# hccho2/Tacotron-Wavenet-Vocoder-Korean

Hardware: AMD Instinct MI355X
Metric: WaveNet autoregressive audio samples/sec at 24 kHz, batch=8 (higher is better)
Workload: dtype f32

## Files before the change

### tacotron-wavenet-vocoder-korean_amd/csrc/twv_wavenet_xcd.hip

```cpp
#include <hip/hip_runtime.h>
#include <stdint.h>
#include <string>
#include <type_traits>
#include "../../include/twv_amd.h"
#include "twv_layout.hpp"
#include "twv_math.hpp"
#include "twv_dev.hpp"
#include "twv_dpp.hpp"
#include "twv_categorical.hpp"
#include "twv_xcd.hpp"

using namespace twv;

#ifndef TWV_CHAIN_PAD
#define TWV_CHAIN_PAD 0
#endif
#ifndef TWV_WATCHDOG_LOG2
#define TWV_WATCHDOG_LOG2 21
#endif
#define TWV_STR2(x) #x
#define TWV_STR(x) TWV_STR2(x)
namespace {

typedef __attribute__((address_space(1))) unsigned long long gu64;
#define LDSU64(i) (((__attribute__((address_space(3))) volatile unsigned long long*)lds)[(i)])

typedef unsigned u32x2v __attribute__((ext_vector_type(2)));
typedef unsigned u32x4s __attribute__((ext_vector_type(4)));
constexpr int kAuxLoad = (int)(16u | 0x80000000u), kAuxStore = 0;
#ifndef TWV_XCD_KF
#define TWV_XCD_KF 1
#endif

__device__ __forceinline__ unsigned long long xb_load(rsrc_t rs, int uword, int lword)
{
    asm volatile("" ::: "memory");
    const u32x2v v = __builtin_amdgcn_raw_buffer_load_b64(rs, lword * 8, uword * 8, kAuxLoad);
    return ((unsigned long long)v.y << 32) | (unsigned long long)v.x;
}
__device__ __forceinline__ u32x4s xb_load2(rsrc_t rs, int uword, int lpair)
{
    asm volatile("" ::: "memory");
    return __builtin_amdgcn_raw_buffer_load_b128(rs, lpair * 16, uword * 8, kAuxLoad);
}
template <bool BAR> __device__ __forceinline__ unsigned long long xb_load_t(rsrc_t rs, int uword, int lword)
{
    if (BAR) asm volatile("" ::: "memory");
    return xb_load(rs, uword, lword);
}
__device__ __forceinline__ unsigned long long xbm_load(rsrc_t rs, int uword, int lword) { return xb_load_t<true>(rs, uword, lword); }
__device__ __forceinline__ u32x4s xbm_load2(rsrc_t rs, int uword, int lpair)
{
    asm volatile("" ::: "memory");
    return xb_load2(rs, uword, lpair);
}
__device__ __forceinline__ void xb_store(rsrc_t rs, int uword, int lword, unsigned tag, float v)
{
    __builtin_amdgcn_raw_buffer_store_b64(u32x2v{__float_as_uint(v), tag}, rs, lword * 8, uword * 8, kAuxStore);
    asm volatile("" ::: "memory");
}
__device__ __forceinline__ void xb_store2(rsrc_t rs, int uword, int lane, unsigned tag, float va, float vb)
{
    const u32x4s d = {__float_as_uint(va), tag, __float_as_uint(vb), tag};
    __builtin_amdgcn_raw_buffer_store_b128(d, rs, lane * 16, uword * 8, kAuxStore);
    asm volatile("s_nop 1" ::"v"(d) : "memory");
}
__device__ __forceinline__ unsigned g_tag(unsigned long long q) { return (unsigned)(q >> 32); }
__device__ __forceinline__ float g_val(unsigned long long q) { return __uint_as_float((unsigned)q); }

struct Poll {
    rsrc_t rs;
    int* status;
    int it;
    bool dead;
};
template <bool BAR = false>
__device__ __forceinline__ bool poll_tick(Poll& p, int code)
{
    if (p.dead) return false;
    if (((++p.it) & 63) == 0) {
        if (xb_load_t<BAR>(p.rs, (int)XcdExch::CTRL + 1, 0) != 0ull) { p.dead = true; return false; }
        if (p.it > (1 << TWV_WATCHDOG_LOG2)) {
            atomicMax(p.status, code);
            xb_store(p.rs, (int)XcdExch::CTRL + 1, 0, 1u, 0.0f);
            p.dead = true;
            return false;
        }
    }
    return true;
}
__device__ __forceinline__ void nap_until(unsigned long long target)
{
#pragma nounroll
    for (int i = 0; i < 4096 && __builtin_amdgcn_s_memtime() < target; ++i) __builtin_amdgcn_s_sleep(8);
}

__device__ __forceinline__ int lane_of_z(int k) { return ((k & 2) ? 16 : 0) + 2 * (k >> 2) + (k & 1); }
__device__ __forceinline__ int lane_of_x(int j) { return j < 16 ? j : 16 + j; }

struct ChainRegs { float wc[32]; float bd; };
__device__ __forceinline__ void dot32_dpp_chain_lo(const float (&w)[16], float xa, float init, float (&c)[4])
{
    float c0 = init, c1, c2, c3;
    asm volatile(
        "s_nop 1\n" TWV_ALIGN8
        "v_fmac_f32_dpp %0, %4, %5 row_newbcast:0 row_mask:0xf bank_mask:0xf\n"
        "v_mul_f32_dpp %1, %4, %6 row_newbcast:1 row_mask:0xf bank_mask:0xf\n"
        "v_mul_f32_dpp %2, %4, %7 row_newbcast:2 row_mask:0xf bank_mask:0xf\n"
        "v_mul_f32_dpp %3, %4, %8 row_newbcast:3 row_mask:0xf bank_mask:0xf\n"
        "v_fmac_f32_dpp %0, %4, %9 row_newbcast:4 row_mask:0xf bank_mask:0xf\n"
        "v_fmac_f32_dpp %1, %4, %10 row_newbcast:5 row_mask:0xf bank_mask:0xf\n"
        "v_fmac_f32_dpp %2, %4, %11 row_newbcast:6 row_mask:0xf bank_mask:0xf\n"
        "v_fmac_f32_dpp %3, %4, %12 row_newbcast:7 row_mask:0xf bank_mask:0xf\n"
        "v_fmac_f32_dpp %0, %4, %13 row_newbcast:8 row_mask:0xf bank_mask:0xf\n"
        "v_fmac_f32_dpp %1, %4, %14 row_newbcast:9 row_mask:0xf bank_mask:0xf\n"
        "v_fmac_f32_dpp %2, %4, %15 row_newbcast:10 row_mask:0xf bank_mask:0xf\n"
        "v_fmac_f32_dpp %3, %4, %16 row_newbcast:11 row_mask:0xf bank_mask:0xf\n"
        "v_fmac_f32_dpp %0, %4, %17 row_newbcast:12 row_mask:0xf bank_mask:0xf\n"
        "v_fmac_f32_dpp %1, %4, %18 row_newbcast:13 row_mask:0xf bank_mask:0xf\n"
        "v_fmac_f32_dpp %2, %4, %19 row_newbcast:14 row_mask:0xf bank_mask:0xf\n"
        "v_fmac_f32_dpp %3, %4, %20 row_newbcast:15 row_mask:0xf bank_mask:0xf"
        : "+v"(c0), "=&v"(c1), "=&v"(c2), "=&v"(c3)
        : "v"(xa), "v"(w[0]), "v"(w[1]), "v"(w[2]), "v"(w[3]), "v"(w[4]), "v"(w[5]), "v"(w[6]), "v"(w[7]), "v"(w[8]), "v"(w[9]), "v"(w[10]), "v"(w[11]), "v"(w[12]), "v"(w[13]), "v"(w[14]), "v"(w[15]));
    c[0] = c0; c[1] = c1; c[2] = c2; c[3] = c3;
}
__device__ __forceinline__ float dot32_dpp_chain_hi(const float (&w)[16], float xb, const float (&c)[4])
{
    float c0 = c[0], c1 = c[1], c2 = c[2], c3 = c[3];
    asm volatile(
        TWV_ALIGN8
        "v_fmac_f32_dpp %0, %4, %5 row_newbcast:0 row_mask:0xf bank_mask:0xf\n"
        "v_fmac_f32_dpp %1, %4, %6 row_newbcast:1 row_mask:0xf bank_mask:0xf\n"
        "v_fmac_f32_dpp %2, %4, %7 row_newbcast:2 row_mask:0xf bank_mask:0xf\n"
        "v_fmac_f32_dpp %3, %4, %8 row_newbcast:3 row_mask:0xf bank_mask:0xf\n"
        "v_fmac_f32_dpp %0, %4, %9 row_newbcast:4 row_mask:0xf bank_mask:0xf\n"
        "v_fmac_f32_dpp %1, %4, %10 row_newbcast:5 row_mask:0xf bank_mask:0xf\n"
        "v_fmac_f32_dpp %2, %4, %11 row_newbcast:6 row_mask:0xf bank_mask:0xf\n"
        "v_fmac_f32_dpp %3, %4, %12 row_newbcast:7 row_mask:0xf bank_mask:0xf\n"
        "v_fmac_f32_dpp %0, %4, %13 row_newbcast:8 row_mask:0xf bank_mask:0xf\n"
        "v_fmac_f32_dpp %1, %4, %14 row_newbcast:9 row_mask:0xf bank_mask:0xf\n"
        "v_fmac_f32_dpp %2, %4, %15 row_newbcast:10 row_mask:0xf bank_mask:0xf\n"
        "v_fmac_f32_dpp %3, %4, %16 row_newbcast:11 row_mask:0xf bank_mask:0xf\n"
        "v_fmac_f32_dpp %0, %4, %17 row_newbcast:12 row_mask:0xf bank_mask:0xf\n"
        "v_fmac_f32_dpp %1, %4, %18 row_newbcast:13 row_mask:0xf bank_mask:0xf\n"
        "v_fmac_f32_dpp %2, %4, %19 row_newbcast:14 row_mask:0xf bank_mask:0xf\n"
        "v_fmac_f32_dpp %3, %4, %20 row_newbcast:15 row_mask:0xf bank_mask:0xf"
        : "+v"(c0), "+v"(c1), "+v"(c2), "+v"(c3)
        : "v"(xb), "v"(w[0]), "v"(w[1]), "v"(w[2]), "v"(w[3]), "v"(w[4]), "v"(w[5]), "v"(w[6]), "v"(w[7]), "v"(w[8]), "v"(w[9]), "v"(w[10]), "v"(w[11]), "v"(w[12]), "v"(w[13]), "v"(w[14]), "v"(w[15]));
    return (c0 + c1) + (c2 + c3);
}

#define XSTAMP(cond_, slot_) do { if ((INSTR & 1) && a.prof != nullptr && b == a.prof_stream && t < a.prof_steps && lane == 0 && (cond_)) a.prof[(long long)t * 64 + (slot_)] = wall_clock64(); } while (0)

#define WACC_DECL() unsigned long long wacc_[6] = {0, 0, 0, 0, 0, 0}, w0_ = 0, wt0_ = 0; if (INSTR & 4) wt0_ = __builtin_amdgcn_s_memtime()
#define WACC_T0() do { if (INSTR & 4) w0_ = __builtin_amdgcn_s_memtime(); } while (0)
#define WACC_T1(i_) do { if (INSTR & 4) wacc_[i_] += __builtin_amdgcn_s_memtime() - w0_; } while (0)
constexpr int kTraceStep = 2000;
#define WTRACE(cond_, slot_) do { if ((INSTR & 4) && a.prof != nullptr && t == kTraceStep && (cond_) && lane == 0) a.prof[2048 + (slot_)] = wall_clock64(); } while (0)
#define WACC_OUT(prof_, slot_, wave_) do { if ((INSTR & 4) && (prof_) != nullptr && (slot_) >= 0 && lane == 0) {                 \
        unsigned long long* o_ = (prof_) + (((slot_) * 8 + (wave_)) * 8);                                                        \
        o_[0] = __builtin_amdgcn_s_memtime() - wt0_;                                                                             \
        o_[1] = wacc_[0]; o_[2] = wacc_[1]; o_[3] = wacc_[2]; o_[4] = wacc_[3]; o_[5] = wacc_[4]; o_[6] = wacc_[5]; } } while (0)
#define XMARK(role_, stage_) do { if ((INSTR & 1) && lane == 0) xb_store(rs, (int)XcdExch::MARK + (role_) * 8 + (int)(threadIdx.x >> 6), 0, (unsigned)t + 1u, (float)(stage_)); } while (0)

enum { ROLE_CHAIN = 0, ROLE_SERVICE = 1, ROLE_SKIP0 = 2, ROLE_CONV0 = 10 };
constexpr int kXcdStreamsPerXcd = kXcdStreams / 8;

struct XArgs {
    XcdLaunch p;
    int n_lc_wg, lc_lpw;
    int n_conv1;
    int total_roles;
};

template <int NS> struct XStreams { rsrc_t rs[NS]; int b[NS]; };
__device__ __forceinline__ rsrc_t exch_rsrc(const XcdLaunch& a, int b)
{
    return __builtin_amdgcn_make_buffer_rsrc(a.exch + (long long)b * XcdExch::WORDS, 0, (int)(XcdExch::WORDS * 8), 0x00020000);
}
struct XLazyRs { const XcdLaunch* a; int xcc, ns; __device__ __forceinline__ rsrc_t operator[](int k) const { return exch_rsrc(*a, xcc + 8 * (k < ns ? k : 0)); } };
struct XLazyB { int xcc, ns; __device__ __forceinline__ int operator[](int k) const { return xcc + 8 * (k < ns ? k : 0); } };
template <int NS> struct XStreamsLazy { XLazyRs rs; XLazyB b; };
constexpr int kSkipLdsWords = 32 * 64;
constexpr int kConvLdsFloats = 16 * 64 + 64;

constexpr int kChainLpw = 5;
template <int INSTR, bool ALL, bool FORCED, bool SEG1, bool TWOSEG, int NC, bool ONEHOT = false, bool HEAD = false, bool CONT = false>
__device__ __forceinline__ void chain_role(const XArgs& xa, int b, rsrc_t rs)
{
    const XcdLaunch& a = xa.p;
    const Layout& L = a.lay;
    const int w = __builtin_amdgcn_readfirstlane(threadIdx.x >> 6), lane = threadIdx.x & 63;
    const int NL = L.NL, T = a.T;
    const bool use_bias = L.use_bias != 0, has_gc = L.G > 0, has_lc = L.L > 0;
    constexpr bool forced = FORCED;
    constexpr int kLayerWaves = kXcdSeg0Layers / kChainLpw;
    const int l0 = (SEG1 ? kXcdSeg0Layers : 0) + kChainLpw * w;
    const int lw0 = kChainLpw * w;
    const int cap = (HEAD || w >= kLayerWaves) ? 0 : kChainLpw;
    int nl = NL - l0;
    nl = nl < 0 ? 0 : (nl > cap ? cap : nl);
    const int nlc = NC >= 0 ? NC : nl;
    const bool next_has = (l0 + nl < NL);
    constexpr bool head = HEAD;
    const bool to_seg1 = TWOSEG && !SEG1 && w == kLayerWaves - 1 && next_has;
    constexpr bool two_seg = TWOSEG;
    if (nl == 0 && !head) return;
    const int oc = dpp_conv_out(lane), od = dpp_dense_out(lane);
    const ActCoef coef = act_coef(lane >= 32);
    float* stb = a.state + (long long)b * L.state_stride;
    Poll pl{rs, a.status, 0, false};
    constexpr int O_WD = 2048;
    constexpr int O_WH = kXcdChainHalfTiles;

    float wlo[kChainLpw - 1][16], whi[kChainLpw][16], bdi[kChainLpw];
#pragma unroll
    for (int i = 0; i < kChainLpw; ++i) {
        if (!HEAD && i < nl) {
            const f32x4* src = reinterpret_cast<const f32x4*>(a.P + L.off_xl + (long long)(l0 + i) * kXcdXlFloats) + lane;
#pragma unroll
            for (int q = 0; q < 4; ++q) {
                const f32x4 lo = src[q * 64], hi = src[(4 + q) * 64];
                if (i == 0) LDS4((O_WH >> 2) + (w * 4 + q) * 64 + lane) = lo;
                else { wlo[i > 0 ? i - 1 : 0][4 * q] = lo.x; wlo[i > 0 ? i - 1 : 0][4 * q + 1] = lo.y; wlo[i > 0 ? i - 1 : 0][4 * q + 2] = lo.z; wlo[i > 0 ? i - 1 : 0][4 * q + 3] = lo.w; }
                whi[i][4 * q] = hi.x; whi[i][4 * q + 1] = hi.y; whi[i][4 * q + 2] = hi.z; whi[i][4 * q + 3] = hi.w;
            }
#pragma unroll
            for (int q = 0; q < 4; ++q) LDS4((O_WD >> 2) + ((lw0 + i) * 4 + q) * 64 + lane) = src[(8 + q) * 64];
            const f32x4 v = src[12 * 64];
            bdi[i] = dense_bias_init(lane, use_bias ? v.y : 0.0f);
        }
    }
    float wcz[32];
    float ha = 0.0f, hb = 0.0f, first_in = 0.0f, b2v = 0.0f, s_lnl = 0.0f, s_tq = 0.0f, samp = 0.0f;
    float cp[4] = {0.0f, 0.0f, 0.0f, 0.0f};
    int q_prev = 0, q_valid = 0, samp_q = 0, first_q = 0;
    float w0row = 0.0f;
    double u_next = 0.0;
    const int chx = dpp_dense_out(lane);
    const bool sampler = head && !forced;
    const bool is15 = (lane & 15) == 15;
    auto causal_prepare = [&]() {
        const float t1 = __int_as_float(__builtin_amdgcn_update_dpp(0, __float_as_int(ha), 0x101, 0xf, 0xf, true));
        const float b0 = __int_as_float(__builtin_amdgcn_update_dpp(0, __float_as_int(hb), 0x150, 0xf, 0xf, true));
        ha = is15 ? b0 : t1;
        hb = __int_as_float(__builtin_amdgcn_update_dpp(0, __float_as_int(hb), 0x101, 0xf, 0xf, true));
        causal_partial_dpp(wcz, ha, hb, cp);
// ... 354 lines not shown
    Poll pl{rs, a.status, 0, false};
    constexpr int kReg = 4, kLds = BIG ? 3 : 0, kSlots = kReg + kLds;
    const int NLDS = BIG ? (NL > 8 * kReg ? NL - 8 * kReg : 0) : 0;
    int nown = 0, nlds = 0;
#pragma unroll
    for (int i = 0; i < kReg; ++i) if (NLDS + s + 8 * i < NL) nown = i + 1;
#pragma unroll
    for (int j = 0; j < kLds; ++j) if (s + 8 * j < NLDS) nlds = j + 1;
    if (nown == 0 && nlds == 0) return;
    Tile t0[kReg];
    unsigned dil[kSlots], roff[kSlots], pos0[kSlots];
    int lay_of[kSlots];
    float bfg[kSlots], gcv[kSlots];
#pragma unroll
    for (int i = 0; i < kSlots; ++i) {
        dil[i] = 1; roff[i] = 0; pos0[i] = 0; bfg[i] = 0.0f; gcv[i] = 0.0f;
        const bool is_lds = i < kLds;
        const int l = is_lds ? s + 8 * i : NLDS + s + 8 * (i - kLds);
        const bool have = is_lds ? i < nlds : (i - kLds) < nown;
        lay_of[i] = have ? l : -1;
        if (have) {
            const float* src = a.P + L.off_layer0 + (long long)l * L.layer_stride + LayerOff::T0;
            if (is_lds) copy_tile_to_lds(l * (kTile / 4), src, lane);
            else load_tile(t0[i - kLds < 0 ? 0 : i - kLds], src, lane);
            dil[i] = (unsigned)pmeta[l]; roff[i] = (unsigned)pmeta[64 + l]; pos0[i] = (unsigned)ringpos[l];
            if (use_bias) bfg[i] = a.P[L.off_layer0 + (long long)l * L.layer_stride + LayerOff::BFG + lane];
            if (has_gc) gcv[i] = a.cond[XH_WORDS + ((long long)b * NL + l) * 64 + lane];
        }
    }
    auto addend = [&](int i, float pre, float lcv) __attribute__((always_inline)) -> float {
        float v = pre;
        if (use_bias) v = v + bfg[i];
        if (has_gc) v = v + gcv[i];
        if (has_lc) v = v + lcv;
        return v;
    };
    const int n16 = lane & 15;
    auto tap0 = [&](int i, unsigned t, float& xa_, float& xb_) __attribute__((always_inline)) {
        const unsigned slot = ring_slot(pos0[i], t, dil[i]);
        const unsigned long long* p = reinterpret_cast<const unsigned long long*>(ring + roff[i] + slot * 32);
        const unsigned long long qa = __hip_atomic_load((gu64*)(p + (n16 >> 1)), __ATOMIC_RELAXED, __HIP_MEMORY_SCOPE_AGENT);
        const unsigned long long qb = __hip_atomic_load((gu64*)(p + 8 + (n16 >> 1)), __ATOMIC_RELAXED, __HIP_MEMORY_SCOPE_AGENT);
        xa_ = __uint_as_float((n16 & 1) ? (unsigned)(qa >> 32) : (unsigned)qa);
        xb_ = __uint_as_float((n16 & 1) ? (unsigned)(qb >> 32) : (unsigned)qb);
    };
    auto dot_slot = [&](int i, float oa, float ob) __attribute__((always_inline)) -> float {
        if (i < kLds) return dot32_dpp_lds(lay_of[i] * (kTile / 4), lane, oa, ob);
        return dot32_dpp(t0[i - kLds < 0 ? 0 : i - kLds].w, oa, ob);
    };
#pragma unroll
    for (int i = 0; i < kSlots; ++i) {
        if (lay_of[i] >= 0) {
            const int l = lay_of[i];
            float xa_, xb_;
            tap0(i, 0u, xa_, xb_);
            const float pre = dot_slot(i, xa_, xb_);
            const float lcv = has_lc ? stb[L.st_lcprev + l * 64 + lane] : 0.0f;
            xb_store(rs, (int)XcdExch::PG + l * 64, lane, 1u, addend(i, pre, lcv));
        }
    }
    for (int t = 0; t < T && !pl.dead; ++t) {
        asm volatile(".p2align 6");
        const unsigned tag = (unsigned)t + 1u;
#pragma unroll
        for (int i = 0; i < kSlots; ++i) {
            if (lay_of[i] >= 0 && !pl.dead) {
                const int l = lay_of[i];
                const bool more = t + 1 < T;
                float oa = 0.0f, ob = 0.0f;
                if (more && dil[i] > 1) tap0(i, (unsigned)t + 1u, oa, ob);
                XMARK(ROLE_SERVICE, 10 + i);
                unsigned long long qa, qb;
                pl.it = 0;
                for (;;) {
                    qa = xb_load(rs, (int)XcdExch::ZX + l * 128 + 1, n16 * 2);
                    qb = xb_load(rs, (int)XcdExch::ZX + l * 128 + 65, n16 * 2);
                    if (__all(g_tag(qa) == tag && g_tag(qb) == tag)) break;
                    if (!poll_tick(pl, 41)) break;
                    __builtin_amdgcn_s_sleep(8);
                }
                if (pl.dead) break;
                const float xa_ = g_val(qa), xb_ = g_val(qb);
                const unsigned slot = ring_slot(pos0[i], (unsigned)t, dil[i]);
                if (lane < 32) ring[roff[i] + slot * 32 + lane] = lane < 16 ? xa_ : xb_;
                if (more) {
                    if (dil[i] == 1) { oa = xa_; ob = xb_; }
                    const float pre = dot_slot(i, oa, ob);
                    float lcv = 0.0f;
                    XMARK(ROLE_SERVICE, 20 + i);
                    if (has_lc) {
                        const int lw = (int)XcdExch::LCR + (((t + 1) % kXcdLcRing) * kXcdLs + l) * 64;
                        unsigned long long ql;
                        pl.it = 0;
                        for (;;) {
                            ql = xb_load(rs, lw, lane);
                            if (__all(g_tag(ql) == tag + 1u)) break;
                            if (!poll_tick(pl, 42)) break;
                            __builtin_amdgcn_s_sleep(8);
                        }
                        if (pl.dead) break;
                        lcv = g_val(ql);
                    }
                    xb_store(rs, (int)XcdExch::PG + l * 64, lane, tag + 1u, addend(i, pre, lcv));
                }
            }
        }
    }
    if (lane == 0 && !pl.dead) {
#pragma unroll
        for (int i = 0; i < kSlots; ++i)
            if (lay_of[i] >= 0) ringpos[lay_of[i]] = (int)((pos0[i] + (unsigned)T) % dil[i]);
    }
}

template <int INSTR, int NS, bool BIG, int KF = 0>
__device__ __forceinline__ void skip_role(const XArgs& xa, const XStreams<NS>& sx, int g)
{
    const XcdLaunch& a = xa.p;
    const Layout& L = a.lay;
    const int v = __builtin_amdgcn_readfirstlane(threadIdx.x >> 6), lane = threadIdx.x & 63;
    const int NL = L.NL - KF, T = a.T;
    const bool use_bias = L.use_bias != 0;
    Poll pl{sx.rs[0], a.status, 0, false};
    constexpr int kReg = BIG ? 5 : 4, kLds = BIG ? 2 : 0, kSlots = kReg + kLds;
    const int NLDS = BIG ? (NL > 8 * kReg ? NL - 8 * kReg : 0) : 0;
    const int SW = BIG ? NL * 64 : kSkipLdsWords;
    const int o_tile4 = (NS * SW * 2 + 3) >> 2;
    int nown = 0, nlds = 0;
#pragma unroll
    for (int i = 0; i < kReg; ++i) if (NLDS + v + 8 * i < NL) nown = i + 1;
#pragma unroll
    for (int j = 0; j < kLds; ++j) if (v + 8 * j < NLDS) nlds = j + 1;
    if (nown == 0 && nlds == 0) return;
    Tile ws[kReg];
    float bs[kSlots];
#pragma unroll
    for (int i = 0; i < kSlots; ++i) bs[i] = 0.0f;
#pragma unroll
    for (int i = 0; i < kReg; ++i) {
        if (i < nown) {
            const long long lb = L.off_layer0 + (long long)(NLDS + v + 8 * i) * L.layer_stride;
            load_tile(ws[i], a.P + lb + LayerOff::SK + (long long)g * kTile, lane);
            if (use_bias) bs[kLds + i] = a.P[lb + LayerOff::SK + (long long)L.NSJ * kTile + g * 64 + lane];
        }
    }
#pragma unroll
    for (int j = 0; j < kLds; ++j) {
        if (j < nlds) {
            const long long lb = L.off_layer0 + (long long)(v + 8 * j) * L.layer_stride;
            copy_tile_to_lds(o_tile4 + (v + 8 * j) * (kTile / 4), a.P + lb + LayerOff::SK + (long long)g * kTile, lane);
            if (use_bias) bs[j] = a.P[lb + LayerOff::SK + (long long)L.NSJ * kTile + g * 64 + lane];
        }
    }
    constexpr bool SPLIT = NS >= 3 && !BIG;
    const int vA = (NL - 1 - NLDS) & 7, vB = (SPLIT && NL >= 2) ? ((NL - 2) & 7) : -1;
    const bool sumA = v == vA, sumB = v == vB, anysum = sumA || sumB;
    Tile wx;
    float bx = 0.0f;
    if (SPLIT && sumB) {
        const long long lb = L.off_layer0 + (long long)(NL - 1) * L.layer_stride;
        load_tile(wx, a.P + lb + LayerOff::SK + (long long)g * kTile, lane);
        if (use_bias) bx = a.P[lb + LayerOff::SK + (long long)L.NSJ * kTile + g * 64 + lane];
    }
    const int n16 = lane & 15;
    const int zc_lane = lane_of_z((lane < 32 ? 0 : 16) + n16);
    unsigned long long seen[kSlots + 1], period = 0;
#pragma unroll
    for (int i = 0; i < kSlots + 1; ++i) seen[i] = 0;
    for (int t = 0; t < T && !pl.dead; ++t) {
        asm volatile(".p2align 6");
        const unsigned tag = (unsigned)t + 1u;
        int nextl[NS];
        float tot[NS];
#pragma unroll
        for (int k = 0; k < NS; ++k) { nextl[k] = 0; tot[k] = 0.0f; }
        auto own_layer = [&](auto&& dot, const float bias, const int l, const int si, const int k0, const int k1) __attribute__((always_inline)) {
            {
                if (!anysum && period) nap_until(seen[si] + period - (period >> 3));
#pragma unroll
                for (int k = 0; k < NS; ++k) {
                    if (pl.dead) break;
                    if (k < k0 || k >= k1) continue;
                    const bool summer = (SPLIT && vB >= 0) ? (k < 2 ? sumA : sumB) : sumA;
                    const rsrc_t rs = sx.rs[k];
                    const int b = sx.b[k];
                    pl.rs = rs;
                    constexpr int kNb = NS >= 3 ? 8 : 1;
                    auto drain = [&](bool blocking) __attribute__((always_inline)) {
                        pl.it = 0;
                        while (nextl[k] < l && !pl.dead) {
                            const int base = nextl[k];
                            unsigned long long q[8];
#pragma unroll
                            for (int j = 0; j < 8; ++j)
                                if (blocking || j < kNb) q[j] = LDSU64(k * SW + (base + j < NL ? base + j : NL - 1) * 64 + lane);
                            bool go = true;
#pragma unroll
                            for (int j = 0; j < 8; ++j) {
                                if (!blocking && j >= kNb) break;
                                go = go && (base + j < l) && __all(g_tag(q[j]) == tag);
                                if (go) { tot[k] = (base + j == 0) ? g_val(q[j]) : tot[k] + g_val(q[j]); nextl[k] = base + j + 1; }
                            }
                            if (nextl[k] == base) {
                                if (!blocking) return;
                                if (!poll_tick(pl, 52)) return;
                            }
                        }
                    };
                    XMARK(ROLE_SKIP0 + g, 10 + si);
                    unsigned long long qz;
                    pl.it = 0;
                    for (;;) {
                        qz = xb_load(rs, (int)XcdExch::ZX + l * 128, zc_lane * 2);
                        if (summer) drain(false);
                        if (__all(g_tag(qz) == tag)) break;
                        if (!poll_tick(pl, 51)) break;
                        if (!summer) __builtin_amdgcn_s_sleep(1);
                    }
                    if ((INSTR & 1) && pl.dead && g == 0 && lane == 0) {
                        xb_store(rs, (int)XcdExch::MARK + 176 + v * 4, 0, g_tag(qz), __uint_as_float(g_tag(qz)));
                        xb_store(rs, (int)XcdExch::MARK + 177 + v * 4, 0, (unsigned)l, __uint_as_float((unsigned)pl.it));
                        xb_store(rs, (int)XcdExch::MARK + 178 + v * 4, 0, tag, __uint_as_float((unsigned)si));
                    }
                    if (!anysum && k == 0) {
                        const unsigned long long now = __builtin_amdgcn_s_memtime();
                        if (si == 0) { const unsigned long long d = now - seen[0]; period = (seen[0] != 0 && d < (1ull << 18)) ? d : 0; }
                        seen[si] = now;
                    }
                    XSTAMP(g == 0 && summer && l == NL - 1, 20);
                    const auto sw = __builtin_amdgcn_permlane32_swap((unsigned)qz, (unsigned)qz, false, false);
                    float val = dot(__uint_as_float(sw[0]), __uint_as_float(sw[1]));
                    if (use_bias) val = val + bias;
                    if (!summer) {
                        LDSU64(k * SW + l * 64 + lane) = ((unsigned long long)tag << 32) | (unsigned long long)__float_as_uint(val);
                    } else {
                        drain(true);
                        tot[k] = (l == 0) ? val : tot[k] + val;
                        nextl[k] = l + 1;
                        if (l == NL - 1 && !pl.dead) {
                            const float h = (KF > 0 || tot[k] > 0.0f) ? tot[k] : 0.0f;
                            xb_store(rs, (int)XcdExch::H1 + g * 64, lane, tag, h);
                            XSTAMP(g == 0, 21);
                        }
                    }
                }
            }
        };
#pragma unroll
        for (int j = 0; j < kLds; ++j) {
            if (j < nlds && !pl.dead)
                own_layer([&](float xa_, float xb_) __attribute__((always_inline)) { return dot32_dpp_lds(o_tile4 + (v + 8 * j) * (kTile / 4), lane, xa_, xb_); }, bs[j], v + 8 * j, j, 0, NS);
        }
#pragma unroll
        for (int i = 0; i < kReg; ++i) {
            if (i < nown && !pl.dead) {
                const int l = NLDS + v + 8 * i;
                own_layer([&](float xa_, float xb_) __attribute__((always_inline)) { return dot32_dpp(ws[i].w, xa_, xb_); }, bs[kLds + i], l, kLds + i, 0,
                          (SPLIT && vB >= 0 && l == NL - 1) ? 2 : NS);
            }
        }
        if (SPLIT && sumB && !pl.dead)
            own_layer([&](float xa_, float xb_) __attribute__((always_inline)) { return dot32_dpp(wx.w, xa_, xb_); }, bx, NL - 1, kSlots, 2, NS);
    }
    if (pl.dead && lane == 0) {
#pragma unroll
        for (int k = 0; k < NS; ++k) xb_store(sx.rs[k], (int)XcdExch::CTRL + 1, 0, 1u, 0.0f);
    }
}

template <int KF, bool BAR>
__device__ __forceinline__ unsigned long long conv1_fetch_h1(Poll& pl, const rsrc_t rs, const int v, const int lane, const unsigned tag, const int last_layer,
                                                             const int zc_lane, const float (&wl)[32], const float bl, const bool use_bias, bool& saw_z)
{
    unsigned long long q;
    pl.it = 0;
    if (KF > 0) {
        unsigned long long qz;
        float val = 0.0f;
        bool havez = false;
        for (;;) {
            if (!havez) qz = xb_load_t<BAR>(rs, (int)XcdExch::ZX + last_layer * 128, zc_lane * 2);
            q = xb_load_t<BAR>(rs, (int)XcdExch::H1 + v * 64, lane);
            if (!havez && __all(g_tag(qz) == tag)) {
                const auto sw = __builtin_amdgcn_permlane32_swap((unsigned)qz, (unsigned)qz, false, false);
                val = dot32_dpp(wl, __uint_as_float(sw[0]), __uint_as_float(sw[1]));
                if (use_bias) val = val + bl;
                havez = true;
                saw_z = true;
            }
            if (havez && __all(g_tag(q) == tag)) break;
            if (!poll_tick<BAR>(pl, 61)) break;
            if (!havez) __builtin_amdgcn_s_sleep(1);
        }
        const float tot = g_val(q) + val;
        const float h = tot > 0.0f ? tot : 0.0f;
        q = (unsigned long long)__float_as_uint(h);
    } else {
        for (;;) {
            q = xb_load_t<BAR>(rs, (int)XcdExch::H1 + v * 64, lane);
            if (__all(g_tag(q) == tag)) break;
            if (!poll_tick<BAR>(pl, 61)) break;
            __builtin_amdgcn_s_sleep(1);
        }
    }
    return q;
}
__device__ __forceinline__ void conv1_load_last_skip(const XcdLaunch& a, const int v, const int lane, Tile& wl, float& bl)
{
    const Layout& L = a.lay;
    const long long lb = L.off_layer0 + (long long)(L.NL - 1) * L.layer_stride;
    load_tile(wl, a.P + lb + LayerOff::SK + (long long)v * kTile, lane);
    if (L.use_bias != 0) bl = a.P[lb + LayerOff::SK + (long long)L.NSJ * kTile + v * 64 + lane];
}
__device__ __forceinline__ void load_half_tile(float (&w)[16], const float* base, const int obase, const int lane)
{
    const float2* p = reinterpret_cast<const float2*>(base + (obase + dpp_dense_out(lane)) * 4 + (((lane >> 4) & 1) ? 2 : 0));
#pragma unroll
    for (int j = 0; j < 8; ++j) {
        const float2 q = p[j * 128];
        w[2 * j] = q.x; w[2 * j + 1] = q.y;
    }
}
__device__ __forceinline__ float conv1d2_chunk_dpp(const float (&t2)[16], const float h)
{
    const float s = dot16_dpp(t2, h);
    const auto ds = __builtin_amdgcn_permlane16_swap(__float_as_uint(s), __float_as_uint(s), false, false);
    return __uint_as_float(ds[0]) + __uint_as_float(ds[1]);
}

template <int INSTR, int NS, bool BAR = false, class SX = XStreams<NS>, int KF = 0>
__device__ __forceinline__ void conv1_role(const XArgs& xa, const SX& sx, int g, const int ns_rt = NS, const int prof_slot = -1)
{
    const XcdLaunch& a = xa.p;
    const Layout& L = a.lay;
    const int v = __builtin_amdgcn_readfirstlane(threadIdx.x >> 6), lane = threadIdx.x & 63;
    const int T = a.T, NCH = L.NCH;
    const bool use_bias = L.use_bias != 0;
    Poll pl{sx.rs[0], a.status, 0, false};
    constexpr int O_PART = 0, O_CNT = 16 * 64;
    if (threadIdx.x < NS) LDSI(threadIdx.x * kConvLdsFloats + O_CNT) = 0;
    __syncthreads();
    const int c0 = 2 * v, c1 = 2 * v + 1;
    Tile ta, tb;
    load_tile(ta, a.P + L.off_w1 + ((long long)g * NCH + c0) * kTile, lane);
    load_tile(tb, a.P + L.off_w1 + ((long long)g * NCH + c1) * kTile, lane);
    const bool summer = v < 2;
    const int hz = 32 * v + dpp_z_index(lane);
    float b1v = 0.0f;
    float t2[16];
    if (summer) {
        if (use_bias) b1v = a.P[L.off_b1 + g * 64 + hz];
        load_half_tile(t2, a.P + L.off_w2 + (long long)(2 * g + v) * kTile, 0, lane);
    }
    Tile wl;
    float bl = 0.0f;
    if (KF > 0) conv1_load_last_skip(a, v, lane, wl, bl);
    const int zc_lane = lane_of_z((lane < 32 ? 0 : 16) + (lane & 15));
    unsigned long long t_arr = 0, period = 0;
    WACC_DECL();
    for (int t = 0; t < T && !pl.dead; ++t) {
        asm volatile(".p2align 6");
        const unsigned tag = (unsigned)t + 1u;
        WACC_T0();
        if (period) nap_until(t_arr + period - (period >> 3));
        WACC_T1(0);
#pragma unroll
        for (int k = 0; k < NS; ++k) {
            if (pl.dead) break;
            if (k >= ns_rt) break;
            const rsrc_t rs = sx.rs[k];
            const int b = sx.b[k];
            const int ob = k * kConvLdsFloats;
            pl.rs = rs;
            XMARK(ROLE_CONV0 + g, 1);
            WACC_T0();
            bool saw_z = false;
            const unsigned long long q = conv1_fetch_h1<KF, BAR>(pl, rs, v, lane, tag, L.NL - 1, zc_lane, wl.w, bl, use_bias, saw_z);
            (void)saw_z;
            WACC_T1(1);
            WTRACE(prof_slot >= 0 && k == 0, 400 + g * 8 + v);
            unsigned long long now_arr = 0;
            if (k == 0) now_arr = __builtin_amdgcn_s_memtime();
            XSTAMP(g == 0 && v == 0, 22);
            const unsigned hq = (unsigned)q;
            const auto p16 = __builtin_amdgcn_permlane16_swap(hq, hq, false, false);
            const auto pa = __builtin_amdgcn_permlane32_swap(p16[0], p16[0], false, false);
            const auto pb = __builtin_amdgcn_permlane32_swap(p16[1], p16[1], false, false);
            float r0, r1;
            dot32_dpp_x2(ta.w, __uint_as_float(pa[0]), __uint_as_float(pb[0]), tb.w, __uint_as_float(pa[1]), __uint_as_float(pb[1]), r0, r1);
            lds[ob + O_PART + c0 * 64 + lane] = r0;
            lds[ob + O_PART + c1 * 64 + lane] = r1;
            asm volatile("" ::: "memory");
            if (lane == 0) __hip_atomic_fetch_add(&LDSI(ob + O_CNT), 1, __ATOMIC_RELAXED, __HIP_MEMORY_SCOPE_WORKGROUP);
            if (k == 0) {
                const unsigned long long d = now_arr - t_arr;
                period = (t_arr != 0 && d < (1ull << 18)) ? d : 0;
                t_arr = now_arr;
            }
            XSTAMP(g == 0 && v == 0, 23);
            XMARK(ROLE_CONV0 + g, 2);
            if (summer) {
                WACC_T0();
                pl.it = 0;
                while (LDSVI(ob + O_CNT) < 8 * (t + 1)) { if (!poll_tick<BAR>(pl, 62)) break; }
                WACC_T1(2);
                asm volatile("" ::: "memory");
                XSTAMP(g == 0 && v == 0, 24);
                float cp[16];
#pragma unroll
                for (int ch = 0; ch < 16; ++ch) cp[ch] = lds[ob + O_PART + ch * 64 + hz];
                __builtin_amdgcn_sched_barrier(0);
                float r = cp[0];
#pragma unroll
                for (int ch = 1; ch < 16; ++ch) r = r + cp[ch];
                if (use_bias) r = r + b1v;
// ... 1460 lines not shown
```

Baseline: 996,900.

## Replace summer-wave skip reduction with chained per-layer LDS accumulation

Changes the skip-connection reduction from one designated summer wave draining all other layers' partial results to a chain. Each layer wave waits on the previous layer's running sum in LDS, adds its own contribution and publishes the new sum, and the last layer writes H1. It adds an inline-asm LDS spin loop that polls for the tag, and it drops the split-summer special case along with its extra weight tile. The aim is to spread the reduction and take the serial drain off the final layer's critical path. The cost is a serial dependency chain across layers within each step.

```diff
diff --git a/tacotron-wavenet-vocoder-korean_amd/csrc/twv_wavenet_xcd.hip b/tacotron-wavenet-vocoder-korean_amd/csrc/twv_wavenet_xcd.hip
--- a/tacotron-wavenet-vocoder-korean_amd/csrc/twv_wavenet_xcd.hip
+++ b/tacotron-wavenet-vocoder-korean_amd/csrc/twv_wavenet_xcd.hip
@@ -93,6 +93,34 @@
 {
 #pragma nounroll
     for (int i = 0; i < 4096 && __builtin_amdgcn_s_memtime() < target; ++i) __builtin_amdgcn_s_sleep(8);
+}
+
+__device__ __forceinline__ unsigned lds_byte_addr_u64(int i)
+{
+    return (unsigned)(unsigned long)(&((__attribute__((address_space(3))) unsigned long long*)lds)[i]);
+}
+__device__ __forceinline__ unsigned long long lds_spin_tag(unsigned byte_addr, unsigned tag, unsigned& left)
+{
+    unsigned long long q;
+    unsigned n;
+    const unsigned long long need = (unsigned long long)tag << 32;
+    asm volatile(
+        "s_movk_i32 %1, 0x1000\n"
+        "1:\n"
+        "ds_read_b64 %0, %2\n"
+        "s_waitcnt lgkmcnt(0)\n"
+        "v_cmp_le_u64 vcc, %3, %0\n"
+        "s_cmp_eq_u64 vcc, exec\n"
+        "s_cbranch_scc1 2f\n"
+        "s_sub_u32 %1, %1, 1\n"
+        "s_cmp_lg_u32 %1, 0\n"
+        "s_cbranch_scc1 1b\n"
+        "2:"
+        : "=&v"(q), "=&s"(n)
+        : "v"(byte_addr), "s"(need)
+        : "vcc", "scc", "memory");
+    left = n;
+    return q;
 }
 
 __device__ __forceinline__ int lane_of_z(int k) { return ((k & 2) ? 16 : 0) + 2 * (k >> 2) + (k & 1); }
@@ -753,115 +781,86 @@
             if (use_bias) bs[j] = a.P[lb + LayerOff::SK + (long long)L.NSJ * kTile + g * 64 + lane];
         }
     }
-    constexpr bool SPLIT = NS >= 3 && !BIG;
-    const int vA = (NL - 1 - NLDS) & 7, vB = (SPLIT && NL >= 2) ? ((NL - 2) & 7) : -1;
-    const bool sumA = v == vA, sumB = v == vB, anysum = sumA || sumB;
-    Tile wx;
-    float bx = 0.0f;
-    if (SPLIT && sumB) {
-        const long long lb = L.off_layer0 + (long long)(NL - 1) * L.layer_stride;
-        load_tile(wx, a.P + lb + LayerOff::SK + (long long)g * kTile, lane);
-        if (use_bias) bx = a.P[lb + LayerOff::SK + (long long)L.NSJ * kTile + g * 64 + lane];
-    }
     const int n16 = lane & 15;
     const int zc_lane = lane_of_z((lane < 32 ? 0 : 16) + n16);
-    unsigned long long seen[kSlots + 1], period = 0;
-#pragma unroll
-    for (int i = 0; i < kSlots + 1; ++i) seen[i] = 0;
+    unsigned long long seen[kSlots], period = 0;
+#pragma unroll
+    for (int i = 0; i < kSlots; ++i) seen[i] = 0;
     for (int t = 0; t < T && !pl.dead; ++t) {
         asm volatile(".p2align 6");
         const unsigned tag = (unsigned)t + 1u;
-        int nextl[NS];
-        float tot[NS];
-#pragma unroll
-        for (int k = 0; k < NS; ++k) { nextl[k] = 0; tot[k] = 0.0f; }
-        auto own_layer = [&](auto&& dot, const float bias, const int l, const int si, const int k0, const int k1) __attribute__((always_inline)) {
+        auto own_layer = [&](auto&& dot, const float bias, const int l, const int si) __attribute__((always_inline)) {
             {
-                if (!anysum && period) nap_until(seen[si] + period - (period >> 3));
+                if (period) nap_until(seen[si] + period - (period >> 3));
+                const bool last = l == NL - 1;
+                const int lp = l > 0 ? l - 1 : 0;
 #pragma unroll
                 for (int k = 0; k < NS; ++k) {
                     if (pl.dead) break;
-                    if (k < k0 || k >= k1) continue;
-                    const bool summer = (SPLIT && vB >= 0) ? (k < 2 ? sumA : sumB) : sumA;
                     const rsrc_t rs = sx.rs[k];
                     const int b = sx.b[k];
                     pl.rs = rs;
-                    constexpr int kNb = NS >= 3 ? 8 : 1;
-                    auto drain = [&](bool blocking) __attribute__((always_inline)) {
-                        pl.it = 0;
-                        while (nextl[k] < l && !pl.dead) {
-                            const int base = nextl[k];
-                            unsigned long long q[8];
-#pragma unroll
-                            for (int j = 0; j < 8; ++j)
-                                if (blocking || j < kNb) q[j] = LDSU64(k * SW + (base + j < NL ? base + j : NL - 1) * 64 + lane);
-                            bool go = true;
-#pragma unroll
-                            for (int j = 0; j < 8; ++j) {
-                                if (!blocking && j >= kNb) break;
-                                go = go && (base + j < l) && __all(g_tag(q[j]) == tag);
-                                if (go) { tot[k] = (base + j == 0) ? g_val(q[j]) : tot[k] + g_val(q[j]); nextl[k] = base + j + 1; }
-                            }
-                            if (nextl[k] == base) {
-                                if (!blocking) return;
-                                if (!poll_tick(pl, 52)) return;
-                            }
-                        }
-                    };
                     XMARK(ROLE_SKIP0 + g, 10 + si);
-                    unsigned long long qz;
+                    unsigned long long qz, qp = 0;
                     pl.it = 0;
                     for (;;) {
                         qz = xb_load(rs, (int)XcdExch::ZX + l * 128, zc_lane * 2);
-                        if (summer) drain(false);
+                        qp = LDSU64(k * SW + lp * 64 + lane);
                         if (__all(g_tag(qz) == tag)) break;
                         if (!poll_tick(pl, 51)) break;
-                        if (!summer) __builtin_amdgcn_s_sleep(1);
+                        if (!last) __builtin_amdgcn_s_sleep(1);
                     }
                     if ((INSTR & 1) && pl.dead && g == 0 && lane == 0) {
                         xb_store(rs, (int)XcdExch::MARK + 176 + v * 4, 0, g_tag(qz), __uint_as_float(g_tag(qz)));
                         xb_store(rs, (int)XcdExch::MARK + 177 + v * 4, 0, (unsigned)l, __uint_as_float((unsigned)pl.it));
                         xb_store(rs, (int)XcdExch::MARK + 178 + v * 4, 0, tag, __uint_as_float((unsigned)si));
                     }
-                    if (!anysum && k == 0) {
+                    XSTAMP(g == 0 && last, 20);
+                    const auto sw = __builtin_amdgcn_permlane32_swap((unsigned)qz, (unsigned)qz, false, false);
+                    float val = dot(__uint_as_float(sw[0]), __uint_as_float(sw[1]));
+                    if (use_bias) val = val + bias;
+                    float tot = val;
+                    if (l > 0) {
+                        asm volatile("" : "+v"(val));
+                        if (!__all(g_tag(qp) == tag)) {
+                            unsigned left;
+                            qp = lds_spin_tag(lds_byte_addr_u64(k * SW + lp * 64 + lane), tag, left);
+                            if (left == 0) {
+                                pl.it = 0;
+                                while (!__all(g_tag(qp) == tag)) {
+                                    if (!poll_tick(pl, 52)) break;
+                                    qp = LDSU64(k * SW + lp * 64 + lane);
+                                }
+                            }
+                        }
+                        tot = g_val(qp) + val;
+                    }
+                    if (pl.dead) break;
+                    if (last) {
+                        const float h = (KF > 0 || tot > 0.0f) ? tot : 0.0f;
+                        xb_store(rs, (int)XcdExch::H1 + g * 64, lane, tag, h);
+                        XSTAMP(g == 0, 21);
+                    } else {
+                        LDSU64(k * SW + l * 64 + lane) = ((unsigned long long)tag << 32) | (unsigned long long)__float_as_uint(tot);
+                    }
+                    if (k == 0) {
                         const unsigned long long now = __builtin_amdgcn_s_memtime();
                         if (si == 0) { const unsigned long long d = now - seen[0]; period = (seen[0] != 0 && d < (1ull << 18)) ? d : 0; }
                         seen[si] = now;
                     }
-                    XSTAMP(g == 0 && summer && l == NL - 1, 20);
-                    const auto sw = __builtin_amdgcn_permlane32_swap((unsigned)qz, (unsigned)qz, false, false);
-                    float val = dot(__uint_as_float(sw[0]), __uint_as_float(sw[1]));
-                    if (use_bias) val = val + bias;
-                    if (!summer) {
-                        LDSU64(k * SW + l * 64 + lane) = ((unsigned long long)tag << 32) | (unsigned long long)__float_as_uint(val);
-                    } else {
-                        drain(true);
-                        tot[k] = (l == 0) ? val : tot[k] + val;
-                        nextl[k] = l + 1;
-                        if (l == NL - 1 && !pl.dead) {
-                            const float h = (KF > 0 || tot[k] > 0.0f) ? tot[k] : 0.0f;
-                            xb_store(rs, (int)XcdExch::H1 + g * 64, lane, tag, h);
-                            XSTAMP(g == 0, 21);
-                        }
-                    }
                 }
             }
         };
 #pragma unroll
         for (int j = 0; j < kLds; ++j) {
             if (j < nlds && !pl.dead)
-                own_layer([&](float xa_, float xb_) __attribute__((always_inline)) { return dot32_dpp_lds(o_tile4 + (v + 8 * j) * (kTile / 4), lane, xa_, xb_); }, bs[j], v + 8 * j, j, 0, NS);
+                own_layer([&](float xa_, float xb_) __attribute__((always_inline)) { return dot32_dpp_lds(o_tile4 + (v + 8 * j) * (kTile / 4), lane, xa_, xb_); }, bs[j], v + 8 * j, j);
         }
 #pragma unroll
         for (int i = 0; i < kReg; ++i) {
-            if (i < nown && !pl.dead) {
-                const int l = NLDS + v + 8 * i;
-                own_layer([&](float xa_, float xb_) __attribute__((always_inline)) { return dot32_dpp(ws[i].w, xa_, xb_); }, bs[kLds + i], l, kLds + i, 0,
-                          (SPLIT && vB >= 0 && l == NL - 1) ? 2 : NS);
-            }
-        }
-        if (SPLIT && sumB && !pl.dead)
-            own_layer([&](float xa_, float xb_) __attribute__((always_inline)) { return dot32_dpp(wx.w, xa_, xb_); }, bx, NL - 1, kSlots, 2, NS);
+            if (i < nown && !pl.dead)
+                own_layer([&](float xa_, float xb_) __attribute__((always_inline)) { return dot32_dpp(ws[i].w, xa_, xb_); }, bs[kLds + i], NLDS + v + 8 * i, kLds + i);
+        }
     }
     if (pl.dead && lane == 0) {
 #pragma unroll
```

After: 1.011 million, median of 6. 1.4% higher.
